# Janmajayamall/tfhe-research

Measured on AMD Instinct MI355X. Metric: programmable_bootstraps_per_sec, higher is better.
Workload: dtype f64

## Files before the change

tfhe-research_amd/csrc/field_fft.h:

```cpp
#pragma once
#include <float.h>
#include <math.h>

#if defined(TFHE_FFT_TRACK_ERROR) && !defined(__HIPCC__)
#include <atomic>
#endif
#include <vector>

#include "platform.h"

namespace tfhe {

struct alignas(16) cplx {
  double re, im;
};

#if defined(TFHE_FFT_TRACK_ERROR) && !defined(__HIPCC__)
inline std::atomic<double>& fft_error_slot() {
  static std::atomic<double> worst{0.0};
  return worst;
}
inline void fft_track_error(double t) {
  const double e = fabs(t - rint(t));
  std::atomic<double>& w = fft_error_slot();
  double cur = w.load(std::memory_order_relaxed);
  while (e > cur && !w.compare_exchange_weak(cur, e, std::memory_order_relaxed)) {
  }
}
#endif

#if defined(TFHE_FFT_TRACK_ERROR) && defined(__HIPCC__)
static __device__ unsigned long long g_fft_margin_bits = 0ull;
__device__ __forceinline__ void fft_track_error_device(double t) {
  const double e = fabs(t - rint(t));
  unsigned long long bits;
  __builtin_memcpy(&bits, &e, sizeof(bits));
  if (bits > __atomic_load_n(&g_fft_margin_bits, __ATOMIC_RELAXED)) atomicMax(&g_fft_margin_bits, bits);
}
#endif

struct FftField {
  typedef cplx elem;
  static constexpr int kParts = 2;
  static constexpr int kId = 5;
  static constexpr int kLogShrink = 1;
  static constexpr int kCoeffs = 2;
  static constexpr int kInverseSweepEvery = 0;
  static constexpr bool kReduceSpectrum = false;
  template <int E>
  static constexpr bool split_accum() { return false; }
  TFHE_HD static elem accum_init() { return elem{0.0, 0.0}; }
  TFHE_HD static void mac(elem, elem, elem&, elem&) {}
  TFHE_HD static elem mac_finish(elem a, elem) { return a; }
  static constexpr int kMaxRows = 1 << 10;
  static constexpr double kMaxError = 0.25;

  TFHE_HD static elem zero() { return elem{0.0, 0.0}; }
  TFHE_HD static void butterfly_forward(elem u, elem b, elem w, elem& y0, elem& y1) {
    const double re = __builtin_fma(-b.im, w.im, __builtin_fma(b.re, w.re, u.re));
    const double im = __builtin_fma(b.im, w.re, __builtin_fma(b.re, w.im, u.im));
    y0 = elem{re, im};
    y1 = elem{__builtin_fma(2.0, u.re, -re), __builtin_fma(2.0, u.im, -im)};
  }
  TFHE_HD static void butterfly_inverse(elem u, elem v, elem w, elem& y0, elem& y1) {
    const double dre = u.re - v.re, dim = u.im - v.im;
    y0 = elem{u.re + v.re, u.im + v.im};
    y1 = elem{__builtin_fma(dre, w.re, dim * w.im), __builtin_fma(dim, w.re, -(dre * w.im))};
  }
  static constexpr bool kPreloadTwiddles = true;
  static constexpr bool kFusedMac = true;
  TFHE_HD static elem mul_add(elem d, elem k, elem acc) {
    return elem{__builtin_fma(-d.im, k.im, __builtin_fma(d.re, k.re, acc.re)),
                __builtin_fma(d.im, k.re, __builtin_fma(d.re, k.im, acc.im))};
  }
  TFHE_HD static constexpr int inverse_twiddle_index(int h, int i) { return h + i; }
  static constexpr int kSmallBits = 31;
  static constexpr int kMaxLogBase = 16;
  static constexpr bool kFuseFirstTwo = false;
  TFHE_HD static void radix4_small(elem&, elem&, elem&, elem&, elem, elem, elem, elem, elem) {}
  TFHE_HD static elem radix8_small_v(elem, elem, elem, elem, elem, elem, elem, elem) { return zero(); }
  TFHE_HD static elem reduce(elem x) { return x; }
  TFHE_HD static elem before_inverse(elem a) { return a; }
  TFHE_HD static elem from_digits(const u32 (&d)[kCoeffs]) { return elem{(double)(i32)d[0], (double)(i32)d[1]}; }
  TFHE_HD static double key_half(u32 w, int part) {
    const i32 lo = (i32)(int16_t)(w & 0xFFFFu);
    if (part == 0) return (double)lo;
    return (double)((i32)(w - (u32)lo) >> 16);
  }
  TFHE_HD static elem from_key_words(const u32 (&w)[kCoeffs], int part) {
    return elem{key_half(w[0], part), key_half(w[1], part)};
  }
  TFHE_HD static elem scale_key(elem x, elem n_inv) { return elem{x.re * n_inv.re, x.im * n_inv.re}; }
  TFHE_HD static u32 to_u32(double t) {
#if defined(TFHE_FFT_TRACK_ERROR) && !defined(__HIPCC__)
    fft_track_error(t);
#elif defined(TFHE_FFT_TRACK_ERROR) && defined(__HIP_DEVICE_COMPILE__)
    fft_track_error_device(t);
#endif
    const double shifted = t + 6755399441055744.0;
    u64 bits;
    __builtin_memcpy(&bits, &shifted, sizeof(bits));
    return (u32)bits;
  }
  TFHE_HD static void finish(const elem (&parts)[kParts], u32 (&out)[kCoeffs]) {
    out[0] = to_u32(parts[0].re) + (to_u32(parts[1].re) << 16);
    out[1] = to_u32(parts[0].im) + (to_u32(parts[1].im) << 16);
  }

  static inline void fill_twiddles(int logm, elem* out) {
    const int m = 1 << logm;
#if !defined(__HIP_DEVICE_COMPILE__)
    static_assert(LDBL_MANT_DIG >= 64, "twiddles are rounded from a 64-bit-mantissa long double");
#endif
    const long double pi = 3.14159265358979323846264338327950288L;
    out[0] = elem{1.0, 0.0};
    for (int s = 0; (1 << s) < m; ++s) {
      const int h = 1 << s;
      for (int i = 0; i < h; ++i) {
        int rev = 0;
        for (int b = 0; b < s; ++b) rev |= ((i >> b) & 1) << (s - 1 - b);
        const long double angle = pi * (long double)(1 + 4 * rev) / (long double)(4 * h);
        out[h + i] = elem{(double)cosl(angle), (double)sinl(angle)};
      }
    }
    for (int i = 0; i < 18; ++i) out[m + i] = elem{0.0, 0.0};
  }
  static inline elem n_inv(int logm) { return elem{1.0 / (double)(1 << logm), 0.0}; }
  static inline double error_bound(int log_n, int rows, int log_base) {
    const double u = 1.1102230246251565e-16, eta = 7.1 * u;
    const double m = (double)(1 << (log_n - 1)), n = (double)(log_n - 1), r = (double)rows;
    const double x = 1.4142135623730951 * (double)(1u << log_base), y = 1.4142135623730951 * 32768.0;
    return 1.001 * (3.0 * n * eta + 1.42 * (r + 1.0) * u) * r * m * sqrt(m) * x * y;
  }
  static inline double exact_bits() { return 0.0; }
  static inline double key_bits() { return 15.0; }
};

}
```

tfhe-research_amd/csrc/pbs_wave.h:

```cpp
#pragma once
#include <utility>

#include "wave_ntt.h"

namespace tfhe {

template <int V>
struct IntC {
  static constexpr int value = V;
};

template <int I, int END, class F>
TFHE_HD void static_for(F&& f) {
  if constexpr (I < END) {
    f(IntC<I>{});
    static_for<I + 1, END>(f);
  }
}

template <class F, int LOGN, int K>
constexpr int key_layout_e() {
  return (F::kLogShrink == 1 && LOGN == 9 && K == 1) ? 8 : 0;
}

// ... 93 lines not shown

template <int LOGN>
TFHE_HD u32 monomial_coeff(const u32* poly, int j, u32 m) {
  constexpr int N = 1 << LOGN;
  const int deg = (int)(m & (N - 1));
  const u32 flip = (m >> LOGN) & 1u;
  const u32 v = poly[(j - deg) & (N - 1)];
  const u32 negate = flip ^ (u32)(j < deg);
  return negate ? (0u - v) : v;
}

template <int LOGN, int T>
struct RotatingOperand {
  static constexpr int N = 1 << LOGN;
  static constexpr int kCount = N / T;
  static_assert(kCount <= 32 && (T & (T - 1)) == 0, "one bit per coefficient; T a power of two");
#if defined(__HIP_DEVICE_COMPILE__)
  typedef const __attribute__((address_space(3))) u32* LdsWords;
  typedef u32 Words;
  TFHE_HD static Words words_at(const u32* p) { return (u32)(size_t)(LdsWords)p; }
  TFHE_HD static u32 read(Words negated, Words kept, u32 s, int index) {
    return ((LdsWords)(size_t)((negated & s) | (kept & ~s)))[index];
  }
#else
  typedef const u32* Words;
  TFHE_HD static Words words_at(const u32* p) { return p; }
  TFHE_HD static u32 read(Words negated, Words kept, u32 s, int index) { return (s ? negated : kept)[index]; }
#endif
  const u32* own;
  Words negated, kept;
  u32 signs;
  TFHE_HD RotatingOperand() {}
  TFHE_HD RotatingOperand(const u32* acc, int lane, u32 m) {
    const int deg = (int)(m & (u32)(N - 1));
    const bool flip = ((m >> LOGN) & 1u) != 0;
    int log_t = 0;
    while ((1 << log_t) < T) ++log_t;
    const int k = (deg - lane + (T - 1)) >> log_t;
    own = acc + lane;
    const u32* base = own - deg;
    negated = words_at(base + (flip ? 0 : N));
    kept = words_at(base + (flip ? N : 0));
    signs = (u32)(~0ull << k) ^ (flip ? 0u : ~0u);
  }
  TFHE_HD u32 rounded(int r, RoundConsts rc) const {
    u32 s = (u32)((int)(signs << (31 - r)) >> 31);
#if defined(__HIP_DEVICE_COMPILE__)
    asm("" : "+v"(s));
#endif
    const u32 c = (rc.half - own[r * T]) - s;
    return ((read(negated, kept, s, r * T) ^ s) + c) & rc.keep;
  }
};
template <int LOGN, int T, int NS>
struct RotatingOperands {
  const RotatingOperand<LOGN, T>* of;
  TFHE_HD u32 rounded(int s, int r, RoundConsts rc) const { return of[s].rounded(r, rc); }
};
template <class Src, class = u32>
struct reads_rounded : std::false_type {};
template <class Src>
struct reads_rounded<Src, decltype(std::declval<const Src&>().rounded(0, 0, RoundConsts{}))> : std::true_type {};
template <class Src, class = u32>
struct reads_rounded1 : std::false_type {};
template <class Src>
struct reads_rounded1<Src, decltype(std::declval<const Src&>().rounded(0, RoundConsts{}))> : std::true_type {};
template <int T, class Src>
TFHE_HD auto rounded_coeff(const Src& src, int s, int r, int, RoundConsts rc, int) -> decltype(src.rounded(s, r, rc)) {
  return src.rounded(s, r, rc);
}
template <int T, class Src>
TFHE_HD u32 rounded_coeff(const Src& src, int s, int r, int lane, RoundConsts rc, long) {
  return round_value_fast(src(s, r * T + lane), rc);
}
template <int T, class Src>
TFHE_HD auto rounded_coeff(const Src& src, int r, int, RoundConsts rc, int) -> decltype(src.rounded(r, rc)) {
  return src.rounded(r, rc);
}
template <int T, class Src>
TFHE_HD u32 rounded_coeff(const Src& src, int r, int lane, RoundConsts rc, long) {
  return round_value_fast(src(r * T + lane), rc);
}

template <class F, int LOGN, int K, int G, int KEYS, int NS, class Ctx, class Src, class Out, class EndKey>
TFHE_HD void external_product_team_multi(const Ctx& c, const PbsParams& P, const typename F::elem* ggsw,
                                         size_t ggsw_words, Src src, Out out, EndKey end_of_key) {
  typedef typename F::elem elem;
  static_assert(KEYS == 1 || NS == 1, "several keys or several samples, not both");
  constexpr int LT = LOGN - F::kLogShrink;
  constexpr int E = NttShape<LT, G>::kE;
  constexpr int EC = NttShape<LOGN, G>::kE;
  constexpr int CO = F::kCoeffs;
  static_assert(EC == E * CO, "coefficients per lane");
  constexpr int T = NttShape<LOGN, G>::kThreads;
  constexpr int N = 1 << LT;
  constexpr int PARTS = F::kParts;
  const int lane = c.tid();
  const int me = c.group();
  constexpr bool SPLIT = F::template split_accum<E>() && KEYS == 1 && NS == 1;
  constexpr int ACCS = KEYS * PARTS;

  elem accum[NS][ACCS][E];
  elem accum_lo[SPLIT ? ACCS : 1][SPLIT ? E : 1];
#pragma unroll
  for (int s = 0; s < NS; ++s)
#pragma unroll
    for (int q = 0; q < ACCS; ++q)
#pragma unroll
      for (int r = 0; r < E; ++r) {
        accum[s][q][r] = SPLIT ? F::accum_init() : F::zero();
        if (SPLIT) accum_lo[SPLIT ? q : 0][SPLIT ? r : 0] = F::zero();
      }

  constexpr bool CARRY_REG = reads_rounded<Src>::value;
  TopConsts<F, LT, G, true> ftop;
  ftop.issue(c.twiddles_uniform());
  u32 v[NS][EC], carry[NS][CARRY_REG ? EC : 1];
  const RoundConsts rc = round_consts(P.ignored_bits);
  const u32 half_base = 1u << (P.log_base - 1);
#pragma unroll
  for (int s = 0; s < NS; ++s)
#pragma unroll
    for (int r = 0; r < EC; ++r) v[s][r] = rounded_coeff<T>(src, s, r, lane, rc, 0);
  ftop.ready();

  constexpr int kChunkRegisters = 8;
  constexpr int TILES = (K + 1) * ACCS;
  constexpr int CH_MAX = kChunkRegisters * 8 / (int)sizeof(elem) / (NS > 1 ? 2 : 1);
  constexpr int CH = E < CH_MAX ? E : CH_MAX;
  constexpr int CHUNKS = TILES * (E / CH);
  auto tile_ptr = [&](u32 level, int sp, int a) -> const elem* {
    const int m = a / PARTS, q = a % PARTS;
    if (TFHE_PROBE_HOT_KEY) return ggsw;
    return ggsw + (size_t)m * ggsw_words + (((size_t)(sp * P.levels + level) * (K + 1) + me) * PARTS + q) * N;
  };
  const bool two = NS == 1 && c.exchange_buffers() == 2;
  elem kbuf[2][CH];
  constexpr bool OWN = F::kLogShrink == 1 && NS == 1 && G == 1 && !SPLIT;
  constexpr bool OWN_REGS = OWN;
  constexpr bool LATE = OWN;
  auto source_of = [&](int sp) -> int {
    if (!OWN) return sp;
    const int at = me + sp;
    return at > K ? at - (K + 1) : at;
  };
  auto load_chunk = [&](u32 level, auto ci_c, int buf) {
    constexpr int ci = decltype(ci_c)::value;
    constexpr int PIECES = E / CH;
    constexpr int q = ci % ACCS, r0 = ((ci / ACCS) % PIECES) * CH, src_poly = ci / (ACCS * PIECES);
    const elem* tile = tile_ptr(level, source_of(src_poly), q);
#pragma unroll
    for (int r = 0; r < CH; ++r)
      kbuf[buf][r] = tile[TFHE_PROBE_HOT_KEY ? (lane & 63) + r : spectrum_slot<LT, G, (int)sizeof(elem), key_layout_e<F, LOGN, K>()>(lane, r0 + r)];
  };
  auto buffers_of_level = [&](u32 t, Ctx (&cl)[NS]) {
#pragma unroll
    for (int s = 0; s < NS; ++s) cl[s] = c.with_exchange_buffer(NS > 1 ? s : (two ? (int)(t & 1u) : 0));
  };
#pragma unroll 1
  for (u32 t = 0; t < P.levels; ++t) {
    const u32 level = P.levels - 1 - t;
    const u32 shift = P.first_shift + P.log_base * t;
    Ctx cl[NS];
    buffers_of_level(t, cl);
    static_for<0, 1>([&](auto pre_c) { load_chunk(level, pre_c, decltype(pre_c)::value); });
    c.compiler_fence();
    constexpr int FS = 1;
    const u32 carry_width = (t == 0) ? 0u : 1u;
    elem own[OWN_REGS ? NS : 1][OWN_REGS ? E : 1];
#pragma unroll
    for (int s0 = 0; s0 < NS; s0 += FS) {
      elem work[FS][E];
      if constexpr (CARRY_REG) {
        if (t == 0) {
#pragma unroll
          for (int s = 0; s < FS; ++s)
#pragma unroll
            for (int r = 0; r < E; ++r) {
              u32 dg[CO];
#pragma unroll
              for (int q = 0; q < CO; ++q) dg[q] = decompose_limb_reg<false>(v[s0 + s][r + q * E], shift, P.log_base, half_base, carry[s0 + s][CARRY_REG ? r + q * E : 0]);
// ... 438 lines not shown
      for (int r = 0; r < E; ++r) d[r] = spec[exchange_slot<LT, 1>(lane, r)];
#pragma unroll
      for (int r = 0; r < E; ++r) accum[r] = F::mul_add(d[r], ring.slot[m % RING_ROWS][r], accum[r]);
      c.compiler_fence();
      if constexpr (m + RING_ROWS < R) ring.template load<m + RING_ROWS>(ggsw, me, q, lane);
      else ring.template load<m + RING_ROWS - R>(ggsw_next, me, q, lane);
    });
  } else {
#pragma unroll 1
    for (u32 level = 0; level < levels; ++level) {
      static_for<0, CHK>([&](auto ci_c) {
        constexpr int ci = decltype(ci_c)::value;
        constexpr int sp = ci / PIECES, r0 = (ci % PIECES) * CH;
        constexpr int cur = ci % 2;
        static_assert(CHK % 2 == 0, "an even number of chunks per level keeps the buffer parity static");
        if constexpr (ci + 1 < CHK) {
          load_chunk(level, IntC<ci + 1>{}, (ci + 1) % 2);
        } else {
          if (level + 1u < levels) load_chunk(level + 1u, IntC<0>{}, 0);
        }
        const elem* spec = c.row_buffer((int)((u32)sp * levels + level));
        elem d[CH];
#pragma unroll
        for (int r = 0; r < CH; ++r) d[r] = spec[exchange_slot<LT, 1>(lane, r0 + r)];
        c.compiler_fence();
#pragma unroll
        for (int r = 0; r < CH; ++r) accum[r0 + r] = F::mul_add(d[r], kbuf[RINGED ? 0 : cur][RINGED ? 0 : r], accum[r0 + r]);
      });
    }
  }

#pragma unroll
  for (int r = 0; r < E; ++r) accum[r] = F::before_inverse(accum[r]);
  itop.ready();
  ntt_inverse<F, LT, 1>(c, accum, itop);
#pragma unroll
  for (int r = 0; r < E; ++r) {
    out(q, r * T + lane, F::to_u32(accum[r].re));
    out(q, (r + E) * T + lane, F::to_u32(accum[r].im));
  }
}

template <class F, int LOGN, int K, int LEVELS = 0, int RING = 0, class Ctx>
TFHE_HD void blind_rotate_team_wide(const Ctx& c, const PbsParams& P, const u32* lwe , const u32* tv ,
                                    const typename F::elem* bsk , u32 i_begin, u32 i_end,
                                    const u32* resume ) {
  constexpr int N = 1 << LOGN;
  constexpr int EC = N / 64;
  const int lane = c.tid();
  const int me = c.group();
  const int q = c.half();
  u32* acc = c.acc();
  const u32 levels = LEVELS > 0 ? (u32)LEVELS : P.levels;
  const size_t ggsw_words = (size_t)(K + 1) * levels * (K + 1) * 2 * (N >> 1);
  typename std::conditional<(LEVELS > 0), WideKeyRing<F, LOGN, K, (LEVELS > 0 ? LEVELS : 1), (RING > 0 ? RING : 1)>, NoKeyRing>::type ring;
  if constexpr (LEVELS > 0) {
    if (i_begin < i_end) ring.prime(bsk + (size_t)i_begin * ggsw_words, me, q, lane);
  }
  if (i_begin > 0) {
    const u32* from = resume + (size_t)me * N;
#pragma unroll
    for (int r = 0; r < EC / 2; ++r) acc[(r + q * (EC / 2)) * 64 + lane] = from[(r + q * (EC / 2)) * 64 + lane];
  } else {
    const RotateInit ri = rotate_init<LOGN>(P, lwe[P.n]);
    rotate_init_fill<LOGN, K, EC / 2>(P, ri, tv, me, acc, [&](int r) { return (r + q * (EC / 2)) * 64 + lane; });
  }
  c.team_sync();
#pragma unroll 1
  for (u32 i = i_begin; i < i_end; ++i) {
    const u32 a_tilde = c.uniform(switch_modulus_2n(lwe[i], LOGN));
    auto src = [&](int j) -> u32 { return monomial_coeff<LOGN>(acc, j, a_tilde) - acc[j]; };
    auto out = [&](int half, int j, u32 value) { c.lds_add(acc + j, value << (16 * half)); };
    const typename F::elem* ggsw = bsk + (size_t)i * ggsw_words;
    const typename F::elem* ggsw_next = i + 1 < i_end ? ggsw + ggsw_words : ggsw;
    if constexpr (short_hot_loop<F, LOGN, K, 1, 1>()) {
      external_product_team_wide<F, LOGN, K, LEVELS>(c, P, ggsw, ggsw_next, ring, RotatingOperand<LOGN, 64>(acc, lane, a_tilde), out);
    } else {
      external_product_team_wide<F, LOGN, K, LEVELS>(c, P, ggsw, ggsw_next, ring, src, out);
    }
    c.team_sync();
  }
}

template <class F, int LOGN, class Ctx, class Src, class Out>
TFHE_HD void external_product_pair(const Ctx& c, const PbsParams& P, const typename F::elem* ggsw, Src src, Out out) {
  typedef typename F::elem elem;
  static_assert(F::kParts == 2 && F::kLogShrink == 1 && F::kCoeffs == 2, "the complex transform: two key parts, two coefficients per element");
  constexpr int K = 1;
  constexpr int LT = LOGN - 1;
  constexpr int G = 0;
  constexpr int E = NttShape<LT, G>::kE;
  constexpr int EC = 2 * E;
  constexpr int T = NttShape<LT, G>::kThreads;
  constexpr int N = 1 << LT;
  const int tid = c.tid();
  const int me = c.group();

  elem accum[2][E];
#pragma unroll
  for (int q = 0; q < 2; ++q)
#pragma unroll
    for (int r = 0; r < E; ++r) accum[q][r] = F::zero();

  TopConsts<F, LT, G, true> ftop;
  ftop.issue(c.twiddles_uniform());
  u32 v[EC], carry[EC];
  const RoundConsts rc = round_consts(P.ignored_bits);
  const u32 half_base = 1u << (P.log_base - 1);
#pragma unroll
  for (int r = 0; r < EC; ++r) v[r] = rounded_coeff<T>(src, r, tid, rc, 0);
  ftop.ready();

  constexpr int CH = 4;
  constexpr int PIECES = E / CH;
  constexpr int CHUNKS = 2 * PIECES * 2;
  elem kbuf[2][CH];
  constexpr int KEY_E = key_layout_e<F, LOGN, 1>();
  static_assert(KEY_E == E, "the prepared key of the pair shape has the pair kernel's layout");
  auto load_chunk = [&](u32 level, auto ci_c, int buf) {
    constexpr int ci = decltype(ci_c)::value;
    constexpr int q = ci % 2, r0 = ((ci / 2) % PIECES) * CH, other = ci / (2 * PIECES);
    const int sp = other ? 1 - me : me;
    const elem* tile = ggsw + ((((size_t)sp * P.levels + level) * (K + 1) + me) * 2 + q) * N;
#pragma unroll
    for (int r = 0; r < CH; ++r) kbuf[buf][r] = tile[spectrum_slot<LT, G, (int)sizeof(elem), KEY_E>(tid, r0 + r)];
  };
#pragma unroll 1
  for (u32 t = 0; t < P.levels; ++t) {
    const u32 level = P.levels - 1 - t;
    const u32 shift = P.first_shift + P.log_base * t;
    load_chunk(level, IntC<0>{}, 0);
    c.compiler_fence();
    elem work[E];
    if (t == 0) {
#pragma unroll
      for (int r = 0; r < E; ++r) {
        u32 dg[2];
        dg[0] = decompose_limb_reg<false>(v[r], shift, P.log_base, half_base, carry[r]);
        dg[1] = decompose_limb_reg<false>(v[r + E], shift, P.log_base, half_base, carry[r + E]);
        work[r] = F::from_digits(dg);
      }
    } else {
#pragma unroll
      for (int r = 0; r < E; ++r) {
        u32 dg[2];
        dg[0] = decompose_limb_reg<true>(v[r], shift, P.log_base, half_base, carry[r]);
        dg[1] = decompose_limb_reg<true>(v[r + E], shift, P.log_base, half_base, carry[r + E]);
        work[r] = F::from_digits(dg);
      }
    }
    ntt_forward<F, LT, G, true, true>(c, work, ftop);
    elem* mine = c.scratch();
#pragma unroll
    for (int r = 0; r < E; ++r) mine[exchange_slot<LT, G>(tid, r)] = work[r];
    c.wave_sync();
    elem d[CH];
    static_for<0, CHUNKS>([&](auto ci_c) {
      constexpr int ci = decltype(ci_c)::value;
      constexpr int q = ci % 2, r0 = ((ci / 2) % PIECES) * CH, other = ci / (2 * PIECES);
      if constexpr (ci + 1 < CHUNKS) load_chunk(level, IntC<ci + 1>{}, (ci + 1) % 2);
      if constexpr (q == 0) {
        if constexpr (other == 0) {
#pragma unroll
          for (int r = 0; r < CH; ++r) d[r] = work[r0 + r];
        } else {
          const elem* spec = c.scratch_of(1 - me);
#pragma unroll
          for (int r = 0; r < CH; ++r) d[r] = spec[exchange_slot<LT, G>(tid, r0 + r)];
        }
      }
      c.compiler_fence();
#pragma unroll
      for (int r = 0; r < CH; ++r) accum[q][r0 + r] = F::mul_add(d[r], kbuf[ci % 2][r], accum[q][r0 + r]);
    });
    c.wave_sync();
  }

  TopConsts<F, LT, G, false> itop;
  itop.issue(c.twiddles_uniform());
#pragma unroll
  for (int r = 0; r < E; ++r) {
    accum[0][r] = F::before_inverse(accum[0][r]);
    accum[1][r] = F::before_inverse(accum[1][r]);
  }
  itop.ready();
  ntt_inverse_pair<F, LT, G>(c, accum[0], accum[1], itop);
#pragma unroll
  for (int r = 0; r < E; ++r) {
    elem parts[2] = {accum[0][r], accum[1][r]};
    u32 vals[2];
    F::finish(parts, vals);
    out(r * T + tid, vals[0]);
    out((r + E) * T + tid, vals[1]);
  }
}

template <class F, int LOGN, class Ctx>
TFHE_HD void blind_rotate_pair(const Ctx& c, const PbsParams& P, const u32* lwe , const u32* tv ,
                               const typename F::elem* bsk , u32 i_begin, u32 i_end,
                               const u32* resume ) {
  constexpr int N = 1 << LOGN;
  constexpr int T = 32;
  constexpr int EC = N / T;
  constexpr int K = 1;
  const int tid = c.tid();
  const int me = c.group();
  u32* acc = c.acc();
  if (i_begin > 0) {
    const u32* from = resume + (size_t)me * N;
#pragma unroll
    for (int r = 0; r < EC; ++r) acc[r * T + tid] = from[r * T + tid];
  } else {
    const RotateInit ri = rotate_init<LOGN>(P, lwe[P.n]);
    rotate_init_fill<LOGN, K, EC>(P, ri, tv, me, acc, [&](int r) { return r * T + tid; });
  }
  c.wave_sync();
  const size_t ggsw_words = (size_t)(K + 1) * P.levels * (K + 1) * 2 * (N >> 1);
#pragma unroll 1
  for (u32 i = i_begin; i < i_end; ++i) {
    const u32 a_tilde = c.uniform(switch_modulus_2n(lwe[i], LOGN));
    const RotatingOperand<LOGN, T> src(acc, tid, a_tilde);
    auto out = [&](int j, u32 value) { c.lds_add(acc + j, value); };
    external_product_pair<F, LOGN>(c, P, bsk + (size_t)i * ggsw_words, src, out);
    c.wave_sync();
  }
}

template <class F, int LOGN, int K, int G, class Ctx>
TFHE_HD void blind_rotate_bmmp_team(const Ctx& c, const PbsParams& P, const u32* lwe ,
                                    const u32* tv ,
                                    const typename F::elem* bsk ) {
  constexpr int E = NttShape<LOGN, G>::kE;
  constexpr int T = NttShape<LOGN, G>::kThreads;
  constexpr int N = 1 << LOGN;
  const int lane = c.tid();
  const int me = c.group();
  u32* acc = c.acc(0);
  {
    const u32 b_tilde = switch_modulus_2n(lwe[P.n], LOGN);
    const u32 m = (2u * N - b_tilde) & (2u * N - 1u);
    const int deg = (int)(m & (N - 1));
    const u32 flip = (m >> LOGN) & 1u;
#pragma unroll
    for (int r = 0; r < E; ++r) {
      const int j = r * T + lane;
      u32 val = 0;
      if (me == K) {
        const u32 t = tv[(j - deg) & (N - 1)] << P.tv_shift;
        val = (flip ^ (u32)(j < deg)) ? (0u - t) : t;
      }
      acc[j] = val;
    }
    c.poly_sync();
  }
  const size_t ggsw_words = (size_t)(K + 1) * P.levels * (K + 1) * F::kParts * (N >> F::kLogShrink);
  u32* stage = reinterpret_cast<u32*>(c.scratch());
#pragma unroll 1
  for (u32 pair = 0; pair < P.n / 2; ++pair) {
    const u32 a0 = c.uniform(switch_modulus_2n(lwe[2 * pair], LOGN));
    const u32 a1 = c.uniform(switch_modulus_2n(lwe[2 * pair + 1], LOGN));
    const u32 e[3] = {(a0 + a1) & (2u * N - 1u), a0, a1};
    auto src = [&](int j) -> u32 { return acc[j]; };
    auto out = [&](int, int j, u32 value) { stage[j] = value; };
    auto end_of_key = [&](int m) {
      c.poly_sync();
#pragma unroll
      for (int r = 0; r < E; ++r) {
        const int j = r * T + lane;
        acc[j] += monomial_coeff<LOGN>(stage, j, e[m]) - stage[j];
      }
      c.poly_sync();
    };
    external_product_team_keys<F, LOGN, K, G, 3>(c, P, bsk + (size_t)pair * 3 * ggsw_words, ggsw_words, src, out,
                                                 end_of_key);
    if (c.exchange_buffers() != 2) c.poly_sync();
  }
}

template <int LOGN, int K, int G, class Ctx>
TFHE_HD void sample_extract_team(const Ctx& c, u32* out , int s = 0) {
  constexpr int E = NttShape<LOGN, G>::kE;
  constexpr int T = NttShape<LOGN, G>::kThreads;
  constexpr int N = 1 << LOGN;
  const int lane = c.tid();
  const int me = c.group();
  const u32* acc = c.acc(s);
  if (me < K) {
#pragma unroll
    for (int r = 0; r < E; ++r) {
      const int x = r * T + lane;
      out[me * N + x] = (x == 0) ? acc[0] : (0u - acc[N - x]);
    }
  } else if (lane == 0) {
    out[K * N] = acc[0];
  }
}

struct CmuxTreePass {
  const void* selectors;
  const void* rot_selectors;
  size_t query_stride;
  u32 tables;
  u32 height;
  u32 log_subtrees;
  u32 shared_sets;
  const u32* even;
// ... 365 lines not shown
```

tfhe-research_amd/csrc/wave_ntt.h:

```cpp
#pragma once
#include <type_traits>

#include "field_fft.h"
#include "field_fp.h"
#include "field_fp49.h"
#include "field_gl.h"

namespace tfhe {

constexpr int ntt_twiddle_words(int n) { return n + 18; }

template <int LOGN, int G = 1>
struct NttShape {
  static_assert(G == 0 || G == 1 || G == 2 || G == 4, "waves per polynomial (0: half a wave)");
  static constexpr int kLogN = LOGN;
  static constexpr int kN = 1 << LOGN;
  static constexpr int kG = G;
  static constexpr int kThreads = G == 0 ? 32 : 64 * G;
  static constexpr int kTBits = (G == 0) ? 5 : (G == 1) ? 6 : (G == 2) ? 7 : 8;
  static constexpr int kEBits = LOGN - kTBits;
  static constexpr int kE = 1 << kEBits;
  static_assert(kEBits >= 2 && kEBits <= 5, "4..32 elements per lane (4: the complex transform at N = 512, four register passes)");
  static constexpr int kPasses = (LOGN + kEBits - 1) / kEBits;
  static_assert(kPasses >= 3 && kPasses <= 5, "three to five register passes");
// ... 259 lines not shown
template <class Elem, int E, int LOW>
__device__ __forceinline__ void swap_transpose(Elem (&x)[E]) {
  static_assert(E == 4, "two-bit windows");
  constexpr int W = (int)(sizeof(Elem) / 4);
  u32 w[E][W];
#pragma unroll
  for (int r = 0; r < E; ++r) __builtin_memcpy(w[r], &x[r], sizeof(Elem));
  exchange_register_bit_with_lane_bit<0, LOW, E, W>(w);
  exchange_register_bit_with_lane_bit<1, LOW + 1, E, W>(w);
#pragma unroll
  for (int r = 0; r < E; ++r) __builtin_memcpy(&x[r], w[r], sizeof(Elem));
}
#endif

template <class Elem, int E>
constexpr bool mac_lowers_priority() {
  return E * (int)sizeof(Elem) == 64;
}

template <class F, int LOGN, int G, int LO_FROM, int LO_TO, bool SKIP_LEAD = false, int NS, class Ctx>
TFHE_HD void ntt_transpose_multi(const Ctx (&c)[NS], typename F::elem (&x)[NS][NttShape<LOGN, G>::kE]) {
  constexpr int E = NttShape<LOGN, G>::kE;
#if defined(__HIP_DEVICE_COMPILE__)
  if constexpr (swap_transpose_shape<LOGN, G, LO_FROM, LO_TO>()) {
    constexpr int LOW = swap_transpose_low_bit<LOGN, G, LO_FROM, LO_TO>();
#pragma unroll
    for (int s = 0; s < NS; ++s) swap_transpose<typename F::elem, E, LOW>(x[s]);
    return;
  }
#endif
  constexpr bool WRITES_CROSS = G > 1 && LO_FROM > 6;
  constexpr bool READS_CROSS = G > 1 && LO_TO > 6;
  static_assert(!(WRITES_CROSS && READS_CROSS), "one of the two windows is a low one");
  const int tid = c[0].tid();
  if (TFHE_PROBE_NO_TRANSPOSE) return;
  if (WRITES_CROSS && !SKIP_LEAD) c[0].poly_sync();
  wave_priority<0>();
#pragma unroll
  for (int s = 0; s < NS; ++s) {
    typename F::elem* buf = c[s].scratch();
#pragma unroll
    for (int r = 0; r < E; ++r) buf[ntt_swizzle<LOGN, G>(ntt_index<LOGN, G, LO_FROM>(tid, r))] = x[s][r];
  }
  if (WRITES_CROSS || READS_CROSS) c[0].poly_sync(); else c[0].wave_sync();
#pragma unroll
  for (int s = 0; s < NS; ++s) {
    const typename F::elem* buf = c[s].scratch();
#pragma unroll
    for (int r = 0; r < E; ++r) x[s][r] = buf[ntt_swizzle<LOGN, G>(ntt_index<LOGN, G, LO_TO>(tid, r))];
  }
  if (READS_CROSS) c[0].poly_sync(); else c[0].wave_sync();
  wave_priority<2>();
}

template <class F, int LOGN, int G, int LO_FROM, int LO_TO, bool SKIP_LEAD = false, class Ctx>
TFHE_HD void ntt_transpose(const Ctx& c, typename F::elem (&x)[NttShape<LOGN, G>::kE]) {
  const Ctx cs[1] = {c};
  ntt_transpose_multi<F, LOGN, G, LO_FROM, LO_TO, SKIP_LEAD, 1>(
      cs, reinterpret_cast<typename F::elem (&)[1][NttShape<LOGN, G>::kE]>(x));
}

template <class F, class = void>
struct PreloadsTwiddles {
  static constexpr bool value = false;
};
template <class F>
struct PreloadsTwiddles<F, decltype((void)F::kPreloadTwiddles)> {
  static constexpr bool value = F::kPreloadTwiddles;
};

template <class F, int LOGN, int G, int LO, bool INVERSE>
TFHE_HD int ntt_low_twiddle_slot(int tid, int b, int i) {
  typedef typename F::elem elem;
  constexpr int e = NttShape<LOGN, G>::kEBits;
  constexpr int H = 1 << (NttShape<LOGN, G>::kTBits - LO);
  const int hi = tid >> LO;
  const int m = NttShape<LOGN, G>::kN >> (b + 1);
  const int cnt = 1 << (LO + e - b - 1);
  constexpr bool TR = ntt_twiddles_transposed<(int)sizeof(elem)>();
  if (!INVERSE || F::kLogShrink) return TR ? m + i * H + hi : m + hi * cnt + i;
  return TR ? m + (cnt - 1 - i) * H + (H - 1 - hi) : 2 * m - 1 - hi * cnt - i;
}

template <class F, int LOGN, int G, int LO, int BHI, int BLO, bool INVERSE>
struct PassTwiddles {
  typedef typename F::elem elem;
  static constexpr int E = NttShape<LOGN, G>::kE;
  static constexpr int count_from(int b) { return b > BHI ? 0 : (E >> (b - LO + 1)) + count_from(b + 1); }
  static constexpr int kCount = count_from(BLO);
  static constexpr int offset(int b) { return count_from(b + 1); }
  elem w[kCount];
  template <class Ctx>
  TFHE_HD void load(const Ctx& c) {
    const elem* tw = c.twiddles();
    const int tid = c.tid();
#pragma unroll
    for (int b = BHI; b >= BLO; --b)
#pragma unroll
      for (int i = 0; i < (E >> (b - LO + 1)); ++i) w[offset(b) + i] = tw[ntt_low_twiddle_slot<F, LOGN, G, LO, INVERSE>(tid, b, i)];
  }
  TFHE_HD elem get(int b, int i) const { return w[offset(b) + i]; }
};
struct NoPassTwiddles {};

template <class F, int LOGN, int G, int LO, int BHI, int BLO, bool SMALL_FIRST, class Ctx, class Top, class Pre = NoPassTwiddles>
TFHE_HD void ntt_pass_forward(const Ctx& c, typename F::elem (&x)[NttShape<LOGN, G>::kE], const Top& top,
                              const Pre& pre = Pre{}) {
  constexpr bool PRE = !std::is_base_of<NoPassTwiddles, Pre>::value;
  typedef typename F::elem elem;
  constexpr int E = NttShape<LOGN, G>::kE;
  constexpr int e = NttShape<LOGN, G>::kEBits;
  constexpr int N = NttShape<LOGN, G>::kN;
  constexpr int H = 1 << (NttShape<LOGN, G>::kTBits - LO);
  const elem* tw = c.twiddles();
  constexpr bool TOP = LO == NttShape<LOGN, G>::kTBits;
  const int hi = c.tid() >> LO;
  constexpr bool FUSE = SMALL_FIRST && F::kFuseFirstTwo && BHI == LOGN - 1 && BHI - BLO >= 1;
  constexpr bool FUSE3 = FUSE && BHI - BLO >= 2;
  if constexpr (FUSE) {
    constexpr int s1 = 1 << (BHI - LO), s2 = s1 >> 1, s3 = s2 >> 1;
    static_assert(!FUSE || TOP, "the fused stages are the top ones");
    const elem w1 = top.tw(1), w2a = top.tw(2), w2b = top.tw(3), w12a = top.fused(0), w12b = top.fused(1);
    if constexpr (FUSE3) {
#pragma unroll
      for (int r = 0; r < s3; ++r) {
        const elem va = x[r + s3], vb = x[r + s3 + s2], vc = x[r + s3 + s1], vd = x[r + s3 + s1 + s2];
        F::radix4_small(x[r], x[r + s2], x[r + s1], x[r + s1 + s2], w1, w2a, w2b, w12a, w12b);
        constexpr int pos[4] = {0, s2, s1, s1 + s2};
#pragma unroll
        for (int q = 0; q < 4; ++q) {
          const elem z = F::radix8_small_v(va, vb, vc, vd, top.fused(2 + 4 * q), top.fused(3 + 4 * q),
                                           top.fused(4 + 4 * q), top.fused(5 + 4 * q));
          const elem u = x[r + pos[q]];
          x[r + pos[q]] = F::add(u, z);
          x[r + pos[q] + s3] = F::sub(u, z);
        }
      }
    } else {
#pragma unroll
      for (int r = 0; r < s2; ++r)
        F::radix4_small(x[r], x[r + s2], x[r + s1], x[r + s1 + s2], w1, w2a, w2b, w12a, w12b);
    }
  }
#pragma unroll
  for (int b = FUSE3 ? BHI - 3 : FUSE ? BHI - 2 : BHI; b >= BLO; --b) {
    const int rb = b - LO;
    const int m = N >> (b + 1);
#pragma unroll
    for (int r0 = 0; r0 < E; ++r0) {
      if ((r0 >> rb) & 1) continue;
      const int r1 = r0 | (1 << rb);
      elem w;
      if constexpr (TOP) w = top.tw(m + (r0 >> (rb + 1)));
      else if constexpr (PRE) w = pre.get(b, r0 >> (rb + 1));
      else w = ntt_twiddles_transposed<(int)sizeof(elem)>() ? tw[m + (r0 >> (rb + 1)) * H + hi]
                                                            : tw[m + (hi << (LO + e - b - 1)) + (r0 >> (rb + 1))];
      const elem u = x[r0];
      if constexpr (FusedForwardButterfly<F>::value) {
        F::butterfly_forward(u, x[r1], w, x[r0], x[r1]);
      } else {
        const elem v = (SMALL_FIRST && b == BHI) ? F::mul_small(x[r1], w) : F::mul(x[r1], w);
        x[r0] = F::add(u, v);
        x[r1] = F::sub(u, v);
      }
    }
  }
}

template <class F, int LOGN, int G, int LO, int BHI, int BLO, class Ctx, class Top, class Pre = NoPassTwiddles>
TFHE_HD void ntt_pass_inverse(const Ctx& c, typename F::elem (&x)[NttShape<LOGN, G>::kE], const Top& top,
                              const Pre& pre = Pre{}) {
  constexpr bool PRE = !std::is_base_of<NoPassTwiddles, Pre>::value;
  typedef typename F::elem elem;
  constexpr int E = NttShape<LOGN, G>::kE;
  constexpr int e = NttShape<LOGN, G>::kEBits;
  constexpr int H = 1 << (NttShape<LOGN, G>::kTBits - LO);
  constexpr bool TOP = LO == NttShape<LOGN, G>::kTBits;
  const elem* tw = c.twiddles();
  const int hi = c.tid() >> LO;
#pragma unroll
  for (int b = BLO; b <= BHI; ++b) {
    const int rb = b - LO;
    const int h = NttShape<LOGN, G>::kN >> (b + 1);
    const int cnt = 1 << (LO + e - b - 1);
#pragma unroll
    for (int r0 = 0; r0 < E; ++r0) {
      if ((r0 >> rb) & 1) continue;
      const int r1 = r0 | (1 << rb);
      elem w;
      if constexpr (TOP) w = top.tw(F::inverse_twiddle_index(h, r0 >> (rb + 1)));
      else if constexpr (PRE) w = pre.get(b, r0 >> (rb + 1));
      else w = ntt_twiddles_transposed<(int)sizeof(elem)>() ? (F::kLogShrink ? tw[h + (r0 >> (rb + 1)) * H + hi]
                                                           : tw[h + (cnt - 1 - (r0 >> (rb + 1))) * H + (H - 1 - hi)])
                                          : (F::kLogShrink ? tw[h + (hi << (LO + e - b - 1)) + (r0 >> (rb + 1))]
                                                           : tw[2 * h - 1 - (hi << (LO + e - b - 1)) - (r0 >> (rb + 1))]);
      const elem u = x[r0];
      const elem v = x[r1];
      if constexpr (FusedForwardButterfly<F>::value) {
        F::butterfly_inverse(u, v, w, x[r0], x[r1]);
      } else {
        x[r0] = F::add(u, v);
        x[r1] = F::mul_inverse(F::sub(v, u), w);
      }
    }
    if (F::kInverseSweepEvery > 0 && (b + 1) % (F::kInverseSweepEvery > 0 ? F::kInverseSweepEvery : 1) == 0 &&
        b + 1 < LOGN) {
#pragma unroll
      for (int r = 0; r < E; ++r) x[r] = F::reduce(x[r]);
    }
  }
}

template <class F, int LOGN, int G, int LO, int BHI, int BLO, bool SMALL, int NS, class Ctx, class Top, class Pre>
TFHE_HD void ntt_pass_forward_each(const Ctx (&c)[NS], typename F::elem (&x)[NS][NttShape<LOGN, G>::kE], const Top& top,
                                   const Pre& pre) {
#pragma unroll
  for (int s = 0; s < NS; ++s) ntt_pass_forward<F, LOGN, G, LO, BHI, BLO, SMALL>(c[s], x[s], top, pre);
}
template <class F, int LOGN, int G, int LO, int BHI, int BLO, int NS, class Ctx, class Top, class Pre>
TFHE_HD void ntt_pass_inverse_each(const Ctx (&c)[NS], typename F::elem (&x)[NS][NttShape<LOGN, G>::kE], const Top& top,
                                   const Pre& pre) {
#pragma unroll
  for (int s = 0; s < NS; ++s) ntt_pass_inverse<F, LOGN, G, LO, BHI, BLO>(c[s], x[s], top, pre);
}

template <class F, int LOGN, int G, int LO, int BHI, int BLO, bool INVERSE, bool PRE>
struct LowPassTwiddles : PassTwiddles<F, LOGN, G, LO, BHI, BLO, INVERSE> {};
template <class F, int LOGN, int G, int LO, int BHI, int BLO, bool INVERSE>
struct LowPassTwiddles<F, LOGN, G, LO, BHI, BLO, INVERSE, false> : NoPassTwiddles {
  template <class Ctx>
  TFHE_HD void load(const Ctx&) {}
};

struct NothingBefore {
  TFHE_HD void operator()() const {}
};
template <class F, int LOGN, int G, bool SMALL_INPUT = false, bool AFTER_BARRIER = false, int NS, class Ctx, class Top,
          class Before = NothingBefore>
TFHE_HD void ntt_forward_multi(const Ctx (&c)[NS], typename F::elem (&x)[NS][NttShape<LOGN, G>::kE], const Top& top,
                               const Before& before_first_store = Before{}) {
  using S = NttShape<LOGN, G>;
  constexpr bool PRE = PreloadsTwiddles<F>::value;
  ntt_pass_forward_each<F, LOGN, G, S::kLo1, LOGN - 1, S::kTBits, SMALL_INPUT>(c, x, top, NoPassTwiddles{});
  LowPassTwiddles<F, LOGN, G, S::kLo2, S::kTBits - 1, S::kLo2, false, PRE> t2;
  t2.load(c[0]);
  before_first_store();
  ntt_transpose_multi<F, LOGN, G, S::kLo1, S::kLo2, AFTER_BARRIER>(c, x);
  ntt_pass_forward_each<F, LOGN, G, S::kLo2, S::kTBits - 1, S::kLo2, false>(c, x, top, t2);
  LowPassTwiddles<F, LOGN, G, S::kLo3, S::kLo2 - 1, S::kLo3, false, PRE> t3;
  t3.load(c[0]);
  ntt_transpose_multi<F, LOGN, G, S::kLo2, S::kLo3>(c, x);
  ntt_pass_forward_each<F, LOGN, G, S::kLo3, S::kLo2 - 1, S::kLo3, false>(c, x, top, t3);
  if constexpr (S::kPasses >= 4) {
    LowPassTwiddles<F, LOGN, G, S::kLo4, S::kLo3 - 1, S::kLo4, false, PRE> t4;
    t4.load(c[0]);
    ntt_transpose_multi<F, LOGN, G, S::kLo3, S::kLo4>(c, x);
    ntt_pass_forward_each<F, LOGN, G, S::kLo4, S::kLo3 - 1, S::kLo4, false>(c, x, top, t4);
  }
  if constexpr (S::kPasses == 5) {
    LowPassTwiddles<F, LOGN, G, S::kLo5, S::kLo4 - 1, 0, false, PRE> t5;
    t5.load(c[0]);
    ntt_transpose_multi<F, LOGN, G, S::kLo4, S::kLo5>(c, x);
    ntt_pass_forward_each<F, LOGN, G, S::kLo5, S::kLo4 - 1, 0, false>(c, x, top, t5);
  }
}

template <class F, int LOGN, int G, bool SMALL_INPUT = false, bool AFTER_BARRIER = false, class Ctx, class Top>
TFHE_HD void ntt_forward(const Ctx& c, typename F::elem (&x)[NttShape<LOGN, G>::kE], const Top& top) {
  const Ctx cs[1] = {c};
  ntt_forward_multi<F, LOGN, G, SMALL_INPUT, AFTER_BARRIER, 1>(
      cs, reinterpret_cast<typename F::elem (&)[1][NttShape<LOGN, G>::kE]>(x), top);
}

template <class F, int LOGN, int G, bool SMALL_INPUT = false, bool AFTER_BARRIER = false, class Ctx>
TFHE_HD void ntt_forward(const Ctx& c, typename F::elem (&x)[NttShape<LOGN, G>::kE]) {
  const TopFromTable<typename F::elem> top{c.twiddles_uniform(), 1 << LOGN};
  ntt_forward<F, LOGN, G, SMALL_INPUT, AFTER_BARRIER>(c, x, top);
}

template <class F, int LOGN, int G, int NS, class Ctx, class Top, class Before = NothingBefore>
TFHE_HD void ntt_inverse_multi(const Ctx (&c)[NS], typename F::elem (&x)[NS][NttShape<LOGN, G>::kE], const Top& top,
                               const Before& before_first_store = Before{}) {
  using S = NttShape<LOGN, G>;
  constexpr bool PRE = PreloadsTwiddles<F>::value;
  if constexpr (S::kPasses == 5) {
    LowPassTwiddles<F, LOGN, G, S::kLo5, S::kLo4 - 1, 0, true, PRE> t5;
    t5.load(c[0]);
    ntt_pass_inverse_each<F, LOGN, G, S::kLo5, S::kLo4 - 1, 0>(c, x, top, t5);
  }
  if constexpr (S::kPasses >= 4) {
    LowPassTwiddles<F, LOGN, G, S::kLo4, S::kLo3 - 1, S::kLo4, true, PRE> t4;
    t4.load(c[0]);
    if constexpr (S::kPasses == 5) {
      before_first_store();
      ntt_transpose_multi<F, LOGN, G, S::kLo5, S::kLo4>(c, x);
    }
    ntt_pass_inverse_each<F, LOGN, G, S::kLo4, S::kLo3 - 1, S::kLo4>(c, x, top, t4);
  }
  LowPassTwiddles<F, LOGN, G, S::kLo3, S::kLo2 - 1, S::kLo3, true, PRE> t3;
  t3.load(c[0]);
  if constexpr (S::kPasses >= 4) {
    if constexpr (S::kPasses == 4) before_first_store();
    ntt_transpose_multi<F, LOGN, G, S::kLo4, S::kLo3>(c, x);
  }
  ntt_pass_inverse_each<F, LOGN, G, S::kLo3, S::kLo2 - 1, S::kLo3>(c, x, top, t3);
  LowPassTwiddles<F, LOGN, G, S::kLo2, S::kTBits - 1, S::kLo2, true, PRE> t2;
  t2.load(c[0]);
  if constexpr (S::kPasses == 3) before_first_store();
  ntt_transpose_multi<F, LOGN, G, S::kLo3, S::kLo2>(c, x);
  ntt_pass_inverse_each<F, LOGN, G, S::kLo2, S::kTBits - 1, S::kLo2>(c, x, top, t2);
  ntt_transpose_multi<F, LOGN, G, S::kLo2, S::kLo1>(c, x);
  ntt_pass_inverse_each<F, LOGN, G, S::kLo1, LOGN - 1, S::kTBits>(c, x, top, NoPassTwiddles{});
}

template <class F, int LOGN, int G, class Ctx, class Top>
TFHE_HD void ntt_inverse(const Ctx& c, typename F::elem (&x)[NttShape<LOGN, G>::kE], const Top& top) {
  const Ctx cs[1] = {c};
  ntt_inverse_multi<F, LOGN, G, 1>(cs, reinterpret_cast<typename F::elem (&)[1][NttShape<LOGN, G>::kE]>(x), top);
}

template <class F, int LOGN, int G, class Ctx>
TFHE_HD void ntt_inverse(const Ctx& c, typename F::elem (&x)[NttShape<LOGN, G>::kE]) {
  const TopFromTable<typename F::elem> top{c.twiddles_uniform(), 1 << LOGN};
  ntt_inverse<F, LOGN, G>(c, x, top);
}

template <class F, int LOGN, int G, class Ctx, class Top, class Before = NothingBefore>
TFHE_HD void ntt_inverse_pair(const Ctx& c, typename F::elem (&a)[NttShape<LOGN, G>::kE],
                              typename F::elem (&b)[NttShape<LOGN, G>::kE], const Top& top,
                              const Before& before_first_store = Before{}) {
  using S = NttShape<LOGN, G>;
  static_assert(G <= 1 && S::kPasses == 3, "wave-local transposes, three passes");
  constexpr bool PRE = PreloadsTwiddles<F>::value;
  LowPassTwiddles<F, LOGN, G, S::kLo3, S::kLo2 - 1, S::kLo3, true, PRE> t3;
  t3.load(c);
  ntt_pass_inverse<F, LOGN, G, S::kLo3, S::kLo2 - 1, S::kLo3>(c, a, top, t3);
  before_first_store();
  ntt_transpose<F, LOGN, G, S::kLo3, S::kLo2>(c, a);
  ntt_pass_inverse<F, LOGN, G, S::kLo3, S::kLo2 - 1, S::kLo3>(c, b, top, t3);
  LowPassTwiddles<F, LOGN, G, S::kLo2, S::kTBits - 1, S::kLo2, true, PRE> t2;
  t2.load(c);
  ntt_transpose<F, LOGN, G, S::kLo3, S::kLo2>(c, b);
  ntt_pass_inverse<F, LOGN, G, S::kLo2, S::kTBits - 1, S::kLo2>(c, a, top, t2);
  ntt_transpose<F, LOGN, G, S::kLo2, S::kLo1>(c, a);
  ntt_pass_inverse<F, LOGN, G, S::kLo2, S::kTBits - 1, S::kLo2>(c, b, top, t2);
  ntt_transpose<F, LOGN, G, S::kLo2, S::kLo1>(c, b);
  ntt_pass_inverse<F, LOGN, G, S::kLo1, LOGN - 1, S::kTBits>(c, a, top, NoPassTwiddles{});
  ntt_pass_inverse<F, LOGN, G, S::kLo1, LOGN - 1, S::kTBits>(c, b, top, NoPassTwiddles{});
}

}
```

Measured before the change: 147,100.

## Keep lowest-window FFT twiddles resident in registers and halve them via rotation

Loads the lowest-pass twiddle set once per blind-rotation loop and reuses it across every external product's forward and inverse transform, instead of reloading per pass. Odd sibling twiddles are now derived as a 90-degree rotation of the even entry, both in the host table and in register-held sets, which halves the twiddle registers per pass. The group index is also made wave-uniform so it can live in a scalar register. The gain in fewer twiddle loads is paid for with more long-lived registers across the loop, which could reduce occupancy. The table change also alters how the odd twiddle values are rounded.

```diff
diff --git a/tfhe-research_amd/csrc/field_fft.h b/tfhe-research_amd/csrc/field_fft.h
--- a/tfhe-research_amd/csrc/field_fft.h
+++ b/tfhe-research_amd/csrc/field_fft.h
@@ -68,6 +68,9 @@
     y1 = elem{__builtin_fma(dre, w.re, dim * w.im), __builtin_fma(dim, w.re, -(dre * w.im))};
   }
   static constexpr bool kPreloadTwiddles = true;
+  static constexpr bool kSiblingTwiddleIsRotation = true;
+  TFHE_HD static elem rotate_twiddle(elem w) { return elem{-w.im, w.re}; }
+  static constexpr bool kScalarGroupIndex = true;
   static constexpr bool kFusedMac = true;
   TFHE_HD static elem mul_add(elem d, elem k, elem acc) {
     return elem{__builtin_fma(-d.im, k.im, __builtin_fma(d.re, k.re, acc.re)),
@@ -117,6 +120,10 @@
     for (int s = 0; (1 << s) < m; ++s) {
       const int h = 1 << s;
       for (int i = 0; i < h; ++i) {
+        if (i & 1) {
+          out[h + i] = rotate_twiddle(out[h + i - 1]);
+          continue;
+        }
         int rev = 0;
         for (int b = 0; b < s; ++b) rev |= ((i >> b) & 1) << (s - 1 - b);
         const long double angle = pi * (long double)(1 + 4 * rev) / (long double)(4 * h);
diff --git a/tfhe-research_amd/csrc/pbs_wave.h b/tfhe-research_amd/csrc/pbs_wave.h
--- a/tfhe-research_amd/csrc/pbs_wave.h
+++ b/tfhe-research_amd/csrc/pbs_wave.h
@@ -199,6 +199,15 @@
   return round_value_fast(src(r * T + lane), rc);
 }
 
+template <class F, class = void>
+struct ScalarGroupIndex {
+  static constexpr bool value = false;
+};
+template <class F>
+struct ScalarGroupIndex<F, decltype((void)F::kScalarGroupIndex)> {
+  static constexpr bool value = F::kScalarGroupIndex;
+};
+
 template <class F, int LOGN, int K, int G, int KEYS, int NS, class Ctx, class Src, class Out, class EndKey>
 TFHE_HD void external_product_team_multi(const Ctx& c, const PbsParams& P, const typename F::elem* ggsw,
                                          size_t ggsw_words, Src src, Out out, EndKey end_of_key) {
@@ -213,7 +222,7 @@
   constexpr int N = 1 << LT;
   constexpr int PARTS = F::kParts;
   const int lane = c.tid();
-  const int me = c.group();
+  const int me = (ScalarGroupIndex<F>::value && G == 1) ? (int)c.uniform((u32)c.group()) : c.group();
   constexpr bool SPLIT = F::template split_accum<E>() && KEYS == 1 && NS == 1;
   constexpr int ACCS = KEYS * PARTS;
 
@@ -818,8 +827,9 @@
   }
 }
 
-template <class F, int LOGN, class Ctx, class Src, class Out>
-TFHE_HD void external_product_pair(const Ctx& c, const PbsParams& P, const typename F::elem* ggsw, Src src, Out out) {
+template <class F, int LOGN, class Ctx, class Src, class Out, class Low = NoPassTwiddles>
+TFHE_HD void external_product_pair(const Ctx& c, const PbsParams& P, const typename F::elem* ggsw, Src src, Out out,
+                                   const Low& low = Low{}) {
   typedef typename F::elem elem;
   static_assert(F::kParts == 2 && F::kLogShrink == 1 && F::kCoeffs == 2, "the complex transform: two key parts, two coefficients per element");
   constexpr int K = 1;
@@ -885,7 +895,7 @@
         work[r] = F::from_digits(dg);
       }
     }
-    ntt_forward<F, LT, G, true, true>(c, work, ftop);
+    ntt_forward<F, LT, G, true, true>(c, work, ftop, low);
     elem* mine = c.scratch();
 #pragma unroll
     for (int r = 0; r < E; ++r) mine[exchange_slot<LT, G>(tid, r)] = work[r];
@@ -920,7 +930,7 @@
     accum[1][r] = F::before_inverse(accum[1][r]);
   }
   itop.ready();
-  ntt_inverse_pair<F, LT, G>(c, accum[0], accum[1], itop);
+  ntt_inverse_pair<F, LT, G>(c, accum[0], accum[1], itop, NothingBefore{}, low);
 #pragma unroll
   for (int r = 0; r < E; ++r) {
     elem parts[2] = {accum[0][r], accum[1][r]};
@@ -951,13 +961,15 @@
     rotate_init_fill<LOGN, K, EC>(P, ri, tv, me, acc, [&](int r) { return r * T + tid; });
   }
   c.wave_sync();
+  typename LowestWindowTwiddles<F, LOGN - 1, 0>::type low;
+  low.load(c);
   const size_t ggsw_words = (size_t)(K + 1) * P.levels * (K + 1) * 2 * (N >> 1);
 #pragma unroll 1
   for (u32 i = i_begin; i < i_end; ++i) {
     const u32 a_tilde = c.uniform(switch_modulus_2n(lwe[i], LOGN));
     const RotatingOperand<LOGN, T> src(acc, tid, a_tilde);
     auto out = [&](int j, u32 value) { c.lds_add(acc + j, value); };
-    external_product_pair<F, LOGN>(c, P, bsk + (size_t)i * ggsw_words, src, out);
+    external_product_pair<F, LOGN>(c, P, bsk + (size_t)i * ggsw_words, src, out, low);
     c.wave_sync();
   }
 }
diff --git a/tfhe-research_amd/csrc/wave_ntt.h b/tfhe-research_amd/csrc/wave_ntt.h
--- a/tfhe-research_amd/csrc/wave_ntt.h
+++ b/tfhe-research_amd/csrc/wave_ntt.h
@@ -365,11 +365,24 @@
   return TR ? m + (cnt - 1 - i) * H + (H - 1 - hi) : 2 * m - 1 - hi * cnt - i;
 }
 
+template <class F, class = void>
+struct SiblingTwiddleIsRotation {
+  static constexpr bool value = false;
+};
+template <class F>
+struct SiblingTwiddleIsRotation<F, decltype((void)F::kSiblingTwiddleIsRotation)> {
+  static constexpr bool value = F::kSiblingTwiddleIsRotation;
+};
+
 template <class F, int LOGN, int G, int LO, int BHI, int BLO, bool INVERSE>
 struct PassTwiddles {
   typedef typename F::elem elem;
   static constexpr int E = NttShape<LOGN, G>::kE;
-  static constexpr int count_from(int b) { return b > BHI ? 0 : (E >> (b - LO + 1)) + count_from(b + 1); }
+  static constexpr bool ROT = SiblingTwiddleIsRotation<F>::value;
+  static constexpr int used(int b) { return E >> (b - LO + 1); }
+  static constexpr bool halved(int b) { return ROT && used(b) >= 2; }
+  static constexpr int held(int b) { return halved(b) ? used(b) / 2 : used(b); }
+  static constexpr int count_from(int b) { return b > BHI ? 0 : held(b) + count_from(b + 1); }
   static constexpr int kCount = count_from(BLO);
   static constexpr int offset(int b) { return count_from(b + 1); }
   elem w[kCount];
@@ -380,9 +393,18 @@
 #pragma unroll
     for (int b = BHI; b >= BLO; --b)
 #pragma unroll
-      for (int i = 0; i < (E >> (b - LO + 1)); ++i) w[offset(b) + i] = tw[ntt_low_twiddle_slot<F, LOGN, G, LO, INVERSE>(tid, b, i)];
-  }
-  TFHE_HD elem get(int b, int i) const { return w[offset(b) + i]; }
+      for (int i = 0; i < held(b); ++i)
+        w[offset(b) + i] = tw[ntt_low_twiddle_slot<F, LOGN, G, LO, INVERSE>(tid, b, halved(b) ? 2 * i : i)];
+  }
+  TFHE_HD elem get(int b, int i) const {
+    if constexpr (ROT) {
+      if (halved(b)) {
+        const elem even = w[offset(b) + (i >> 1)];
+        return (i & 1) ? F::rotate_twiddle(even) : even;
+      }
+    }
+    return w[offset(b) + i];
+  }
 };
 struct NoPassTwiddles {};
 
@@ -515,32 +537,56 @@
   TFHE_HD void load(const Ctx&) {}
 };
 
+template <class F, int LOGN, int G>
+struct LowestWindowTwiddles {
+  using S = NttShape<LOGN, G>;
+  static_assert(F::kLogShrink == 1, "one set for both directions: the inverse butterfly reads the forward entry");
+  static constexpr int kBHi = (S::kPasses == 3 ? S::kLo2 : S::kPasses == 4 ? S::kLo3 : S::kLo4) - 1;
+  typedef PassTwiddles<F, LOGN, G, 0, kBHi, 0, false> type;
+};
+template <class Low>
+constexpr bool has_resident_twiddles() {
+  return !std::is_base_of<NoPassTwiddles, Low>::value;
+}
+
 struct NothingBefore {
   TFHE_HD void operator()() const {}
 };
 template <class F, int LOGN, int G, bool SMALL_INPUT = false, bool AFTER_BARRIER = false, int NS, class Ctx, class Top,
-          class Before = NothingBefore>
+          class Before = NothingBefore, class Low = NoPassTwiddles>
 TFHE_HD void ntt_forward_multi(const Ctx (&c)[NS], typename F::elem (&x)[NS][NttShape<LOGN, G>::kE], const Top& top,
-                               const Before& before_first_store = Before{}) {
+                               const Before& before_first_store = Before{}, const Low& low = Low{}) {
   using S = NttShape<LOGN, G>;
   constexpr bool PRE = PreloadsTwiddles<F>::value;
+  constexpr bool RES = has_resident_twiddles<Low>();
   ntt_pass_forward_each<F, LOGN, G, S::kLo1, LOGN - 1, S::kTBits, SMALL_INPUT>(c, x, top, NoPassTwiddles{});
   LowPassTwiddles<F, LOGN, G, S::kLo2, S::kTBits - 1, S::kLo2, false, PRE> t2;
   t2.load(c[0]);
   before_first_store();
   ntt_transpose_multi<F, LOGN, G, S::kLo1, S::kLo2, AFTER_BARRIER>(c, x);
   ntt_pass_forward_each<F, LOGN, G, S::kLo2, S::kTBits - 1, S::kLo2, false>(c, x, top, t2);
-  LowPassTwiddles<F, LOGN, G, S::kLo3, S::kLo2 - 1, S::kLo3, false, PRE> t3;
-  t3.load(c[0]);
-  ntt_transpose_multi<F, LOGN, G, S::kLo2, S::kLo3>(c, x);
-  ntt_pass_forward_each<F, LOGN, G, S::kLo3, S::kLo2 - 1, S::kLo3, false>(c, x, top, t3);
+  if constexpr (RES && S::kPasses == 3) {
+    ntt_transpose_multi<F, LOGN, G, S::kLo2, S::kLo3>(c, x);
+    ntt_pass_forward_each<F, LOGN, G, S::kLo3, S::kLo2 - 1, S::kLo3, false>(c, x, top, low);
+  } else {
+    LowPassTwiddles<F, LOGN, G, S::kLo3, S::kLo2 - 1, S::kLo3, false, PRE> t3;
+    t3.load(c[0]);
+    ntt_transpose_multi<F, LOGN, G, S::kLo2, S::kLo3>(c, x);
+    ntt_pass_forward_each<F, LOGN, G, S::kLo3, S::kLo2 - 1, S::kLo3, false>(c, x, top, t3);
+  }
   if constexpr (S::kPasses >= 4) {
-    LowPassTwiddles<F, LOGN, G, S::kLo4, S::kLo3 - 1, S::kLo4, false, PRE> t4;
-    t4.load(c[0]);
-    ntt_transpose_multi<F, LOGN, G, S::kLo3, S::kLo4>(c, x);
-    ntt_pass_forward_each<F, LOGN, G, S::kLo4, S::kLo3 - 1, S::kLo4, false>(c, x, top, t4);
+    if constexpr (RES && S::kPasses == 4) {
+      ntt_transpose_multi<F, LOGN, G, S::kLo3, S::kLo4>(c, x);
+      ntt_pass_forward_each<F, LOGN, G, S::kLo4, S::kLo3 - 1, S::kLo4, false>(c, x, top, low);
+    } else {
+      LowPassTwiddles<F, LOGN, G, S::kLo4, S::kLo3 - 1, S::kLo4, false, PRE> t4;
+      t4.load(c[0]);
+      ntt_transpose_multi<F, LOGN, G, S::kLo3, S::kLo4>(c, x);
+      ntt_pass_forward_each<F, LOGN, G, S::kLo4, S::kLo3 - 1, S::kLo4, false>(c, x, top, t4);
+    }
   }
   if constexpr (S::kPasses == 5) {
+    static_assert(!RES || S::kPasses < 5, "no resident set in the five-pass shapes");
     LowPassTwiddles<F, LOGN, G, S::kLo5, S::kLo4 - 1, 0, false, PRE> t5;
     t5.load(c[0]);
     ntt_transpose_multi<F, LOGN, G, S::kLo4, S::kLo5>(c, x);
@@ -548,11 +594,11 @@
   }
 }
 
-template <class F, int LOGN, int G, bool SMALL_INPUT = false, bool AFTER_BARRIER = false, class Ctx, class Top>
-TFHE_HD void ntt_forward(const Ctx& c, typename F::elem (&x)[NttShape<LOGN, G>::kE], const Top& top) {
+template <class F, int LOGN, int G, bool SMALL_INPUT = false, bool AFTER_BARRIER = false, class Ctx, class Top, class Low = NoPassTwiddles>
+TFHE_HD void ntt_forward(const Ctx& c, typename F::elem (&x)[NttShape<LOGN, G>::kE], const Top& top, const Low& low = Low{}) {
   const Ctx cs[1] = {c};
   ntt_forward_multi<F, LOGN, G, SMALL_INPUT, AFTER_BARRIER, 1>(
-      cs, reinterpret_cast<typename F::elem (&)[1][NttShape<LOGN, G>::kE]>(x), top);
+      cs, reinterpret_cast<typename F::elem (&)[1][NttShape<LOGN, G>::kE]>(x), top, NothingBefore{}, low);
 }
 
 template <class F, int LOGN, int G, bool SMALL_INPUT = false, bool AFTER_BARRIER = false, class Ctx>
@@ -608,15 +654,27 @@
   ntt_inverse<F, LOGN, G>(c, x, top);
 }
 
-template <class F, int LOGN, int G, class Ctx, class Top, class Before = NothingBefore>
+template <class Own, class Ctx, class Low>
+TFHE_HD typename std::conditional<has_resident_twiddles<Low>(), const Low&, Own>::type first_pass_twiddles(const Ctx& c, const Low& low) {
+  if constexpr (has_resident_twiddles<Low>()) {
+    return low;
+  } else {
+    Own t;
+    t.load(c);
+    return t;
+  }
+}
+
+template <class F, int LOGN, int G, class Ctx, class Top, class Before = NothingBefore, class Low = NoPassTwiddles>
 TFHE_HD void ntt_inverse_pair(const Ctx& c, typename F::elem (&a)[NttShape<LOGN, G>::kE],
                               typename F::elem (&b)[NttShape<LOGN, G>::kE], const Top& top,
-                              const Before& before_first_store = Before{}) {
+                              const Before& before_first_store = Before{}, const Low& low = Low{}) {
   using S = NttShape<LOGN, G>;
   static_assert(G <= 1 && S::kPasses == 3, "wave-local transposes, three passes");
   constexpr bool PRE = PreloadsTwiddles<F>::value;
-  LowPassTwiddles<F, LOGN, G, S::kLo3, S::kLo2 - 1, S::kLo3, true, PRE> t3;
-  t3.load(c);
+  typename std::conditional<has_resident_twiddles<Low>(), const Low&,
+                            LowPassTwiddles<F, LOGN, G, S::kLo3, S::kLo2 - 1, S::kLo3, true, PRE>>::type t3 = first_pass_twiddles<
+      LowPassTwiddles<F, LOGN, G, S::kLo3, S::kLo2 - 1, S::kLo3, true, PRE>>(c, low);
   ntt_pass_inverse<F, LOGN, G, S::kLo3, S::kLo2 - 1, S::kLo3>(c, a, top, t3);
   before_first_store();
   ntt_transpose<F, LOGN, G, S::kLo3, S::kLo2>(c, a);
```

New measurement: 149,400, median of 6. 1.02x the previous value.
